# smarc-project/smarc_navigation

Measured on AMD Instinct MI355X. Metric: filter steps/sec at 1M particles x 512 MBES beams; pose RMSE vs ref, higher is better.
Workload: dtype f64 state / f32 ray-cast; 1 GPU; 1048576 particles/GPU x 512 beams, 999698-triangle mesh (708x708 height field triangulated) -- RECOGNISED AS A LATTICE by mesh_build: swept on its 708 x 708 node heights, no triangle record is read (an irregular TIN of the same size: value_tin / extra.mesh_tin), predict+MBES update+normalise+systematic resample+mean/cov per step; particles_per_gpu=1048576, beams=512, map=mesh, parallelism=particle-shard x1

## Files before the change

smarc_navigation_amd/csrc/mcl_api.hip:

```cpp
#include "mcl_host.h"
#include "mcl_host_resample.h"
#include "mcl_host_moments.h"
#include "mcl_host_update.h"
#include "mcl_host_landmarks.h"
#include "mcl_host_ranges.h"
#include "mcl_host_step.h"
#include "mcl_host_history.h"
#include "mcl_host_acoustic.h"
#include "mcl_recovery.h"


#include "mcl_dr_impl.h"
#include "mcl_gridmap.h"

extern "C" {

int mcl_abi_version(void) { return MCL_ABI_VERSION; }

const char* mcl_status_string(int s) {
  switch (s) {
    case MCL_OK: return "ok";
    case MCL_ERR_INVALID: return "invalid argument";
    case MCL_ERR_NO_DEVICE: return "no gfx950 HIP device";
    case MCL_ERR_HIP: return "HIP runtime error";
// ... 49 lines not shown
  h->world = cfg->world > 1 ? cfg->world : 1;
  h->rank = h->world > 1 ? cfg->rank : 0;
  h->ng = cfg->n_global > 0 ? cfg->n_global : cfg->n_particles;
  h->goff = h->world > 1 ? cfg->global_offset : 0;
  h->device = cfg->device;
  memset(&h->tacc, 0, sizeof h->tacc);
  {
    auto on = [](const char* name) {
      const char* v = getenv(name);
      return v && v[0] == '1';
    };
    auto env_tristate = [](const char* name) {
      const char* v = getenv(name);
      return !v ? -1 : (v[0] == '1' ? 1 : 0);
    };
    h->env_debug_work = getenv("MCL_DEBUG_WORK") != nullptr;
    h->env_sort = env_tristate("MCL_SORT_VISITS");
    h->env_sweep = env_tristate("MCL_SWEEP");
    h->env_slice = env_tristate("MCL_SLICE");
    h->env_slice_group = env_tristate("MCL_SLICE_GROUP");
    h->env_handover_slice = env_tristate("MCL_HANDOVER_SLICE");
    h->env_visit = env_tristate("MCL_VISIT");
    h->env_sweep_uniform = env_tristate("MCL_SWEEP_UNIFORM");
    if (const char* sv = getenv("MCL_SWEEP_STEP_CAP")) h->env_sweep_step_cap = std::max(0, atoi(sv));
    if (const char* sv = getenv("MCL_VISIT_BINS")) {
      int b[3] = {0, 0, 0};
      if (sscanf(sv, "%d,%d,%d", &b[0], &b[1], &b[2]) == 3 && b[0] >= 1 && b[1] >= 1 && b[2] >= 1 &&
          (long long)b[0] * b[1] * b[2] <= VISIT_MAX_BINS && (b[0] * b[1] * b[2]) % 64 == 0)
        for (int c = 0; c < 3; ++c) h->visit_nb[c] = b[c];
    }
    if (const char* sv = getenv("MCL_VISIT_RANGE")) {
      const double r = atof(sv);
      if (r >= 0.5 && r <= 16.0) h->visit_range = (float)r;
    }
    if (const char* sv = getenv("MCL_VISIT_MIN_N")) h->visit_min_n = std::max(1ll, atoll(sv));
    if (const char* sv = getenv("MCL_SWEEP_NSUB")) h->env_nsub = (sv[0] == '2' || sv[0] == '4') ? sv[0] - '0' : 1;
    h->env_force_comm = on("MCL_FORCE_COMM");
    if (const char* ex = getenv("MCL_EXCHANGE")) h->exch_allgather = strcmp(ex, "allgather") == 0;
    if (const char* fi = getenv("MCL_FAULT_INJECT")) h->fault_step = strcmp(fi, "step_after_predict") == 0;
    h->env_no_overlap = on("MCL_NO_OVERLAP");
  }
  if (h->ng > 0xffffffffll || h->goff + h->n > h->ng || h->rank >= h->world) {
    g_create_err = "mcl_create: inconsistent shard geometry";
    delete h;
    return MCL_ERR_INVALID;
  }
// ... 1185 lines not shown
```

smarc_navigation_amd/csrc/mcl_host.h:

```cpp
#pragma once
#include <hip/hip_runtime.h>
#include <rccl/rccl.h>

#include <rocprim/device/device_radix_sort.hpp>

#include <chrono>
#include <cmath>
#include <cstdlib>
#include <cstdio>
#include <cstring>
#include <string>
#include <thread>
#include <vector>

#include "../../include/mcl.h"
#include "mcl_host_pure.h"
#include "mcl_kernels.h"
#include "mcl_mbes.h"
#include "mcl_sweep.h"
#include "mcl_slice.h"
#include "mcl_mesh.h"
#include "mcl_resample.h"
#include "mcl_resample_alt.h"
#include "mcl_landmarks.h"
// ... 84 lines not shown
  DevBuf<int> dupes;
  DevBuf<double> cs, chunk, uni_dev;
  long long residual_k = -1;
  bool idx_explicit = false;
  int beams_cap = 0;
  std::vector<float> beam_cache;
  int beam_lo = -1, beam_hi = -1;
  bool beams_sorted = false;
  std::vector<float> ranges_host;
  bool sweep_angles_ok = false;
  int b_split = 0;
  int sweep_cap = 0;
  DevBuf<float> sweep_buf[2];
  PinBuf<float> sweep_stage[2];
  hipEvent_t ev_stage[2] = {nullptr, nullptr};
  bool stage_used[2] = {false, false};
  int sweep_sel = 0;
  hipStream_t copy_stream = nullptr;
  DevBuf<u32> defer_idx;
  DevBuf<u32> defer2_idx;
  int env_handover_slice = -1;
  int env_sweep_step_cap = 0;
  int env_sweep_uniform = -1;
  DevBuf<unsigned long long> sweep_work_dev;
  DevBuf<unsigned> reasons_dev;
  DevBuf<u32> visit_okey, visit_base;
  DevBuf<unsigned short> visit_cnt;
  DevBuf<u64> visit_desc;
  u32 visit_epoch = 0;
  DevBuf<VisitPar> visit_par;
  unsigned visit_flip = 0;
  bool gather_attr_set = false;
  bool visit_ready = false;
  bool pose_visit = false;
  int env_visit = -1;
  int visit_nb[3] = {16, 32, 8};
  float visit_range = 2.5f;
  long long visit_min_n = 393216;
  int env_sweep = -1;
  int env_nsub = 0;
  bool sweep_now = false;
  bool slice_now = false;
  bool handover_slice_now = false;
  int env_slice = -1;
  int env_slice_group = -1;
  DevBuf<u32> slice_loose;
// ... 287 lines not shown
```

smarc_navigation_amd/csrc/mcl_host_update.h:

```cpp
#pragma once
#include "mcl_host_moments.h"

namespace {

int upload_beams(mcl_handle* h, const float* ranges, const float* beam_angles, int B) {
  h->det_ride = nullptr;
  h->det_ride_dev = nullptr;
  if (B > h->beams_cap) {
    h->beams_cap = 0;
    h->beam_cache.clear();
    RESERVE(h, h->beam_sc, (size_t)B);
    RESERVE(h, h->ranges_dev, (size_t)B);
    h->beams_cap = B;
  }
  if ((int)h->beam_cache.size() != B || memcmp(h->beam_cache.data(), beam_angles, sizeof(float) * B) != 0) {
    std::vector<float2> sc(B);
    for (int b = 0; b < B; ++b) {
      sc[b].x = (float)std::sin((double)beam_angles[b]);
      sc[b].y = (float)std::cos((double)beam_angles[b]);
    }
    RET_IF(upload(h, h->beam_sc, sc.data(), sizeof(float2) * (size_t)B));
    h->beam_cache.assign(beam_angles, beam_angles + B);
    int lo = 0, hi = 0;
    bool finite = true;
// ... 385 lines not shown
void cast_slice_handovers(mcl_handle* h, int dgrid, const MbesArgs& d) {
  k_mbes_cast<1, EXPECT, 2><<<dgrid, MBES_THREADS, 0, h->stream>>>(d);
}

int allow_slice_group_lds(mcl_handle* h, size_t lds_g) {
  if (h->slice_attr_set && lds_g <= h->slice_attr_bytes) return MCL_OK;
  HIPCHK(h, hipFuncSetAttribute((const void*)k_mbes_slice_group, hipFuncAttributeMaxDynamicSharedMemorySize, (int)lds_g));
  h->slice_attr_set = true;
  h->slice_attr_bytes = lds_g;
  return MCL_OK;
}

struct SweepGrid {
  int sgrid, sthreads, dgrid;
  size_t lds;
};

template <int SURF, int MAP>
void launch_sweep(mcl_handle* h, const MbesPlan& p, const SweepGrid& g, const MbesArgs& a, const MbesArgs& d) {
  if (p.with_ranges) {
    t_begin(h, MCL_K_MBES_MAIN);
    if (p.nsub > 1)
      k_mbes_sweep<SURF, false, true><<<g.sgrid, g.sthreads, g.lds, h->stream>>>(a);
    else if ((SURF == 2 || SURF == 3) && a.sweep_work)
      k_mbes_sweep_work<(SURF == 3 ? 3 : 2)><<<g.sgrid, SWEEP_THREADS, g.lds, h->stream>>>(a);
    else
      k_mbes_sweep<SURF, false><<<g.sgrid, SWEEP_THREADS, g.lds, h->stream>>>(a);
    t_end(h);
    k_mbes_cast<MAP, false, 2><<<g.dgrid, MBES_THREADS, 0, h->stream>>>(d);
  } else {
    k_mbes_sweep<SURF, true><<<g.sgrid, SWEEP_THREADS, g.lds, h->stream>>>(a);
    k_mbes_cast<MAP, true, 2><<<g.dgrid, MBES_THREADS, 0, h->stream>>>(d);
  }
}

bool staged_handover(const mcl_handle* h, const MbesPlan& p) {
  return p.with_ranges && p.nsub == 1 && h->map_kind == 1 && !p.structured && h->mesh->tin_holes && h->mesh->cell_tri &&
         h->env_slice != 0 && h->env_handover_slice != 0;
}
int run_staged_handover(mcl_handle* h, const MbesPlan& p, const SweepGrid& g, const MbesArgs& a, MbesArgs d, const MbesCounters& wh) {
  const int B = p.B;
  RESERVE(h, h->defer2_idx, (size_t)h->n);
  const long long ngr = (h->n + SLICE_G - 1) / SLICE_G;
  RESERVE(h, h->slice_loose, (size_t)ngr);
  t_begin(h, MCL_K_MBES_MAIN);
  if (h->mesh->tin_rims)
    k_mbes_sweep<6, false><<<g.sgrid, SWEEP_THREADS, g.lds, h->stream>>>(a);
  else
// ... 18 lines not shown
    s2.slice_loose_count = (int*)(h->ctrl + CTRL_LOOSE);
    k_mbes_slice_group<<<(unsigned)std::min<long long>(ngr, hgrid), SLICE_G_THREADS, lds_g, h->stream>>>(s2);
  }
  k_mbes_slice<false><<<pgrid, SLICE_THREADS, slice_lds_bytes(B), h->stream>>>(s2);
  d.perm = h->defer2_idx;
  d.n_dev = s2.defer_count;
  cast_slice_handovers<false>(h, g.dgrid, d);
  return MCL_OK;
}

void debug_sweep_handovers(mcl_handle* h, const MbesArgs& a) {
  int cnt = 0;
  (void)hipMemcpyAsync(&cnt, a.defer_count, sizeof(int), hipMemcpyDeviceToHost, h->stream);
  (void)hipStreamSynchronize(h->stream);
  unsigned long long shared = 0, steps = 0;
  if (a.sweep_work) {
    unsigned long long w[64];
    (void)hipMemcpy(w, a.sweep_work, sizeof w, hipMemcpyDeviceToHost);
    for (int k = 0; k < 64; ++k) {
      shared += w[k] >> 32;
      steps += w[k] & 0xffffffffull;
    }
  }
  fprintf(stderr, "[mbes] sweep handed over %d of %lld particles (clamp to r_max %s); wave walk steps shared %llu of %llu\n", cnt,
          (long long)h->n, a.sweep_noclamp ? "proved idle: skipped" : "kept", shared, steps);
#ifdef SWEEP_REASONS
  unsigned why[16];
  (void)hipMemcpy(why, h->reasons_dev, sizeof why, hipMemcpyDeviceToHost);
  (void)hipMemset(h->reasons_dev, 0, sizeof why);
  fprintf(stderr, "[mbes] declined sides by reason:");
  for (int k = 0; k < 16; ++k)
    if (why[k]) fprintf(stderr, " %d:%u", k, why[k]);
  fprintf(stderr, "\n");
#endif
}

int run_sweep(mcl_handle* h, const MbesPlan& p, MbesArgs& a, const MbesCounters& wh) {
  a.sweep_noclamp = sweep_noclamp(h, p) ? 1 : 0;
  a.sweep_uniform = h->env_sweep_uniform == 1 ? 1 : 0;
  a.sweep_step_cap = h->env_sweep_step_cap;
  a.sweep_work = nullptr;
  if (h->env_debug_work) {
    RESERVE(h, h->sweep_work_dev, 64);
    HIPCHK(h, hipMemsetAsync(h->sweep_work_dev, 0, 64 * sizeof(unsigned long long), h->stream));
    a.sweep_work = h->sweep_work_dev;
  }
  SweepGrid g;
  g.sthreads = p.nsub == 4 ? 512 : SWEEP_THREADS;
  const int per_block = g.sthreads / 64 / (2 * p.nsub) * 64;
  g.sgrid = (int)((p.n_part + per_block - 1) / per_block);
  g.lds = sweep_lds_bytes(p.B);
  g.dgrid = handover_cast_grid(p, wh);
  const MbesArgs d = handover_cast_args(a, wh);
  const bool staged = staged_handover(h, p);
  if (p.with_ranges) h->handover_slice_now = staged;
  if (staged)
    RET_IF(run_staged_handover(h, p, g, a, d, wh));
  else if (h->map_kind == 0)
    launch_sweep<0, 0>(h, p, g, a, d);
  else if (!p.structured && h->mesh->tin_rims)
    launch_sweep<6, 1>(h, p, g, a, d);
  else if (!p.structured)
    launch_sweep<5, 1>(h, p, g, a, d);
// ... 223 lines not shown
```

smarc_navigation_amd/csrc/mcl_mbes.h:

```cpp
#pragma once
#include <hip/hip_fp16.h>

#include "mcl_device.h"
#include "mcl_kernels.h"

#ifndef MBES_WAVES
#define MBES_WAVES 8
#endif
#ifndef MBES_MIN_WAVES_PER_SIMD
#define MBES_MIN_WAVES_PER_SIMD 8
#endif
#ifndef MBES_MIN_WAVES_MESH
#define MBES_MIN_WAVES_MESH 6
#endif
#define MBES_THREADS (MBES_WAVES * 64)
#ifndef MBES_TILE_FLOATS
#define MBES_TILE_FLOATS 8192
#endif
#ifndef MBES_DIR_BINS
#define MBES_DIR_BINS 16
#endif
#ifndef MBES_DIR_BINS
#define MBES_DIR_BINS 16
#endif
// ... 26 lines not shown
  u32 tin_he_bytes;
  const u32* cell_rim;
  u32 tin_outline;
  u32 tin_nhe;
  const float4* cell_tri;
  double x0, y0;
};

struct MbesArgs {
  const double* st[6];
  long long n;
  double m2o[12];
  double off_t[3];
  double off_R[9];
  MbesPose* pose;
  const float2* beam_sc;
  const float* ranges;
  int n_beams;
  int sorted;
  int b_lo, b_hi;
  const float* grid;
  const float* grid_pad;
  int nyp;
  int nx, ny;
  double ox, oy, inv_res;
  float res;
  float zmin_map, zmax_map;
  int cells;
  int diag_mode;
  float inv_sigma, r_max;
  double lognorm;
  double* lw;
  u64* max_slots;
  float* exp_out;
  long long exp_first, exp_count;
  MeshArgs mesh;
  const u32* perm;
  struct MbesGroup* groups;
  int* worklist;
  int* work_count;
  unsigned long long* stats;
  const float4* sweep_beams;
  const float* sweep_tail_run;
  const float* sweep_tan0;
  const float* sweep_tail;
  int b_split;
// ... 891 lines not shown
```

smarc_navigation_amd/csrc/mcl_mesh.h:

```cpp
#pragma once
#include <algorithm>
#include <cmath>
#include <cstring>
#include <string>
#include <unordered_map>
#include <vector>

#include "../../include/mcl.h"
#include "mcl_halfedge.h"
#include "mcl_mbes.h"

struct MeshDev {
  DevBuf<float4> tri;
  DevBuf<float4> tri_mt;
  DevBuf<u32> cell_start;
  DevBuf<uint2> cell_info;
  int gx = 0, gy = 0;
  double x0 = 0, y0 = 0, cs = 1;
  float zmin = 0, zmax = 0;
  size_t n_records = 0;
  DevBuf<float> heights;
  DevBuf<float> heights_pad;
  size_t n_vertical = 0;
  int diag_mode = 0;
  double slope_max = 0;
  DevBuf<uint4> tin_he;
  size_t tin_he_bytes = 0;
  bool tin_ok = false;
  size_t tin_nhe = 0;
  size_t tin_outline = 0;
  size_t tin_rims = 0;
  DevBuf<u32> cell_rim;
  bool tin_holes = false;
  DevBuf<float4> cell_tri;
};

inline size_t padded_heights_count(int nx, int ny) { return ((size_t)nx + 2) * ((size_t)ny + 2); }
inline hipError_t upload_padded_heights(const float* z, int nx, int ny, float* out) {
  const size_t nyp = (size_t)ny + 2, cnt = padded_heights_count(nx, ny);
  std::vector<float> pad(cnt);
  auto nanp = [](uint32_t payload) {
    const uint32_t b = 0x7fc00000u | payload;
    float f;
    memcpy(&f, &b, 4);
    return f;
  };
  for (size_t i = 0; i < (size_t)nx + 2; ++i)
    for (size_t j = 0; j < nyp; ++j) {
      const bool ox = i == 0 || i == (size_t)nx + 1, oy = j == 0 || j == nyp - 1;
      pad[i * nyp + j] = (ox || oy) ? nanp((ox ? 1u : 0u) | (oy ? 2u : 0u)) : z[(i - 1) * (size_t)ny + (j - 1)];
    }
  return hipMemcpy(out, pad.data(), sizeof(float) * cnt, hipMemcpyHostToDevice);
}

inline void mesh_free(MeshDev* m) { delete m; }

inline float half_bits_to_float(uint16_t h) {
  const uint32_t sign = (uint32_t)(h & 0x8000u) << 16, exp = (h >> 10) & 0x1fu, man = h & 0x3ffu;
  uint32_t bits;
  if (exp == 0) {
    if (man == 0) {
      bits = sign;
    } else {
      float f = (float)man * 5.9604644775390625e-08f;
      memcpy(&bits, &f, 4);
      bits |= sign;
    }
  } else if (exp == 31) {
    bits = sign | 0x7f800000u | (man << 13);
  } else {
    bits = sign | ((exp + 112u) << 23) | (man << 13);
  }
  float out;
  memcpy(&out, &bits, 4);
  return out;
// ... 373 lines not shown
            const u32 dbit = (ix < (size_t)m->gx && iy < (size_t)m->gy) ? diag[ix * m->gy + iy] : 0u;
            b = (b & ~1u) | dbit;
            memcpy(&hts[ix * nny + iy], &b, 4);
          }
      {
        double g2 = 0.0;
        for (size_t ix = 0; ix + 1 < nnx; ++ix)
          for (size_t iy = 0; iy + 1 < nny; ++iy) {
            const double h00 = hts[ix * nny + iy], h10 = hts[(ix + 1) * nny + iy], h01 = hts[ix * nny + iy + 1],
                         h11 = hts[(ix + 1) * nny + iy + 1];
            const double ax = std::max(std::fabs(h10 - h00), std::fabs(h11 - h01));
            const double ay = std::max(std::fabs(h01 - h00), std::fabs(h11 - h10));
            g2 = std::max(g2, ax * ax + ay * ay);
          }
        m->slope_max = std::sqrt(g2) / cs;
      }
      if (m->heights.reserve(hts.size()) != MCL_OK || m->heights_pad.reserve(padded_heights_count((int)nnx, (int)nny)) != MCL_OK ||
          hipMemcpy(m->heights, hts.data(), sizeof(float) * hts.size(), hipMemcpyHostToDevice) != hipSuccess ||
          upload_padded_heights(hts.data(), (int)nnx, (int)nny, m->heights_pad) != hipSuccess) {
        *err = "set_map_mesh: device allocation failed";
        mesh_free(m);
        return MCL_ERR_ALLOC;
      }
    }
  }
  if (!m->heights || want_slice) {
    std::vector<float4> ct(3 * std::max<size_t>(m->n_records, 1));
    for (size_t r = 0; r < m->n_records; ++r) {
      const u32 k = rec_tri[r];
      for (int c = 0; c < 3; ++c) {
        const float* v = verts + 3 * (size_t)tris[3 * (size_t)k + c];
        ct[3 * r + c] = make_float4(v[0], v[1], v[2], 0.f);
      }
      memcpy(&ct[3 * r].w, &k, 4);
    }
    if (m->cell_tri.reserve(ct.size()) != MCL_OK ||
        hipMemcpy(m->cell_tri, ct.data(), sizeof(float4) * ct.size(), hipMemcpyHostToDevice) != hipSuccess) {
      (void)hipGetLastError();
      m->cell_tri.reset();
    }
  }
  *out = m;
  return MCL_OK;
}

inline MeshArgs mesh_args(const MeshDev* m) {
// ... 19 lines not shown
```

smarc_navigation_amd/csrc/mcl_sweep.h:

```cpp
#pragma once
#include "mcl_halfedge.h"
#include "mcl_mbes.h"

#ifndef SWEEP_THREADS
#define SWEEP_THREADS 256
#endif
#ifndef SWEEP_MIN_WAVES_GRID
#define SWEEP_MIN_WAVES_GRID 6
#endif
#ifndef SWEEP_MIN_WAVES_TIN
#define SWEEP_MIN_WAVES_TIN 6
#endif
#define SWEEP_TIN_GAPS 12
#ifndef SWEEP_MIN_WAVES
#define SWEEP_MIN_WAVES 8
#endif

#ifdef SWEEP_REASONS
#define SWEEP_NOTE(code) do { if (a.reasons) atomicAdd(&a.reasons[(code) & 15], 1u); } while (0)
#else
#define SWEEP_NOTE(code) ((void)0)
#endif
#define SWEEP_FAIL(code) do { SWEEP_NOTE(code); return false; } while (0)
#ifdef SWEEP_TIMELINE
// ... 97 lines not shown
               : [acc] "+v"(acc), [bp] "+v"(bp),
                 [ep] "=&v"(ep), [d] "=&v"(d), [ec] "=&v"(ec), [e2] "=&v"(e2), [sav] "=&s"(sav), [odd] "=&s"(odd)
               : [dss] "v"(dss), [num] "v"(num), [tp] "v"(tp), [sc] "v"(sc), [tc] "v"(tc), [dts] "v"(dts), [sel] "s"(sel)
               : "vcc", "scc", "v56", "v57", "v58", "v59", "v60", "v61", "v62", "v63");
}

__device__ __forceinline__ float seg_tau(float num, float D, float tp, float tc) {
  return __builtin_amdgcn_fmed3f(num * __builtin_amdgcn_rcpf(D), tp, tc);
}

struct SweepNode {
  int P;
  float d;
  float s, t;
};

__device__ __forceinline__ bool sweep_border_final(const MbesArgs& a, float h, float c2z, float c1x, float c1y) {
  const unsigned side = __float_as_uint(h) & 3u;
  const float sb = fast_sqrt(fmaxf(1.f - c2z * c2z, 0.f));
  const float lhs = sb * (a.sweep_slope + sb), rhs = 0.9f * (c2z - a.sweep_slope * sb);
  return (side == 1u || side == 2u) & (lhs < rhs * fabsf(side == 1u ? c1x : c1y));
}

template <int SURF, bool EXPECT_ONLY, bool SUB = false, bool WORK = false>
__device__ __forceinline__ bool sweep_side(const MbesArgs& a, const MbesPose& P, const float4* __restrict__ sbeam,
                                           const float* __restrict__ stail, int side, int sub, int nsub,
                                           float* __restrict__ exp_row, float& acc_out) {
  acc_out = 0.f;
  const int nx = a.nx, ny = a.ny, B = a.n_beams;
  bool pre = P.um >= 1.0 && P.um < (double)(nx - 2) && P.vm >= 1.0 && P.vm < (double)(ny - 2);
  const float c2z = P.c2[2];
  pre = pre & (c2z >= a.sweep_c2z_min);
  const double fum = pre ? floor(P.um) : 1.0, fvm = pre ? floor(P.vm) : 1.0;
  const int I0 = (int)fum, J0 = (int)fvm;
  const float ul = (float)(P.um - fum), vl = (float)(P.vm - fvm);
  const float res = a.res, inv_res = (float)a.inv_res, oz = P.oz;
  const float sg = side ? -1.f : 1.f;
  const int nb_side = side ? a.b_split : B - a.b_split;
  const int per = SUB ? max((nb_side + nsub - 1) / nsub, 2) : nb_side;
  const int first = SUB ? min(sub * per, nb_side) : 0, last = SUB ? min(first + per, nb_side) : nb_side;
  int ptr = side ? a.b_split - 1 - first : a.b_split + first;
  const int pstep = side ? -1 : 1, pend = side ? a.b_split - 1 - last : a.b_split + last;
  const bool none = ptr == pend;
  float s_stop = none ? 0.f : a.r_max;
  if (!none) {
    const float2 sc = a.beam_sc[side ? 0 : B - 1];
    const float dz_e = sc.x * P.c1[2] - sc.y * c2z;
    if (dz_e < -1e-4f) s_stop = fminf(s_stop, (a.zmin_map - oz) * fast_rcp(dz_e) * fabsf(sc.x));
  }
  s_stop += 2.f * res;
  {
    const float rc = fast_rcp(c2z);
    const float sl = fabsf(P.c1[2]) * (s_stop + 2.f * res);
    const float t_hi = ((oz - a.zmin_map) + sl) * rc + res, t_lo = fminf(((oz - a.zmax_map) - sl) * rc - res, 0.f);
    const float s_hi = s_stop + 2.f * res;
    const float ax = sg * P.c1[0] * inv_res, ay = sg * P.c1[1] * inv_res, bx = -P.c2[0] * inv_res, by = -P.c2[1] * inv_res;
    const float fi0 = (float)I0, fj0 = (float)J0;
    const float n0 = fminf(t_lo * bx, t_hi * bx), n1 = fmaxf(t_lo * bx, t_hi * bx);
    const float m0 = fminf(t_lo * by, t_hi * by), m1 = fmaxf(t_lo * by, t_hi * by);
    pre = pre & (fi0 + n0 >= 3.f) & (fi0 + n1 <= (float)(nx - 5)) & (fj0 + m0 >= 3.f) & (fj0 + m1 <= (float)(ny - 5));
    pre = pre & (s_hi * fmaxf(fabsf(ax), fabsf(ay)) + fmaxf(-t_lo, t_hi) * fmaxf(fabsf(bx), fabsf(by)) < 30000.f);
  }
  if (!pre) SWEEP_FAIL(1);
  const int nyp = a.nyp;
  const int g0i = (I0 + 1) * nyp + (J0 + 1);
  const float* __restrict__ gp = a.grid_pad + (size_t)g0i;
  const __amdgpu_buffer_rsrc_t grsrc = __builtin_amdgcn_make_buffer_rsrc((void*)a.grid_pad, 0, (nx + 2) * nyp * 4, 0x00020000);
  const int ny4 = nyp * 4, g0b = g0i * 4;
  float dxs = -P.c2[0], dys = -P.c2[1], dzs = -c2z, r0 = 0.f;
  bool own_start = false;
  if (SUB && first > 0 && !none) {
    const float2 sc = a.beam_sc[ptr];
    dxs = sc.x * P.c1[0] - sc.y * P.c2[0];
    dys = sc.x * P.c1[1] - sc.y * P.c2[1];
    dzs = sc.x * P.c1[2] - sc.y * c2z;
    const float te = dzs < -1e-4f ? fminf(a.r_max, (a.zmin_map - oz) * fast_rcp(dzs) + res) : a.r_max;
    const float ex = te * dxs * inv_res, ey = te * dys * inv_res;
    own_start = ((float)I0 + fminf(ex, 0.f) >= 3.f) & ((float)I0 + fmaxf(ex, 0.f) <= (float)(nx - 5)) &
                ((float)J0 + fminf(ey, 0.f) >= 3.f) & ((float)J0 + fmaxf(ey, 0.f) <= (float)(ny - 5));
    if (!own_start) {
      dxs = -P.c2[0];
      dys = -P.c2[1];
      dzs = -c2z;
    }
  }
  for (int attempt = 0; attempt < 2; ++attempt) {
    r0 = cast_clear<SURF>(gp, nyp, a, ul, vl, oz, dxs * inv_res, dys * inv_res, dzs, a.zmax_map, a.r_max);
    if (!SUB || !own_start || ((r0 < a.r_max) & (r0 > 0.f))) break;
    dxs = -P.c2[0];
    dys = -P.c2[1];
    dzs = -c2z;
    own_start = false;
  }
  if (!(r0 < a.r_max)) SWEEP_FAIL(5);
  if (none) return true;
  const float nx_ = P.c1[1] * P.c2[2] - P.c1[2] * P.c2[1], ny_ = P.c1[2] * P.c2[0] - P.c1[0] * P.c2[2],
              nz_ = P.c1[0] * P.c2[1] - P.c1[1] * P.c2[0];
  const float pu = nx_ * res, pv = ny_ * res, pz = nz_, p0 = -(pu * ul + pv * vl + pz * oz);
  const float su = sg * P.c1[0] * res, sv = sg * P.c1[1] * res, sz = sg * P.c1[2];
  float s0 = -(su * ul + sv * vl + sz * oz);
  const float tu = -P.c2[0] * res, tv = -P.c2[1] * res, tz = -c2z, t0 = -(tu * ul + tv * vl + tz * oz);
  auto node = [&](int Pk) {
    SweepNode N;
    N.P = Pk;
    const int j = __builtin_amdgcn_sbfe(Pk, 0, 16), i = (Pk - j) >> 16;
    const float h = gp[i * nyp + j];
    const float fi = (float)i, fj = (float)j;
    N.d = fmaf(pu, fi, fmaf(pv, fj, fmaf(pz, h, p0)));
    N.s = fmaf(su, fi, fmaf(sv, fj, fmaf(sz, h, s0)));
    N.t = fmaf(tu, fi, fmaf(tv, fj, fmaf(tz, h, t0)));
    return N;
  };
  SweepNode A, Bn;
  int C;
  float s_prev, t_prev, s_cur, t_cur;
  {
    const float uh = fmaf(r0, dxs * inv_res, ul), vh = fmaf(r0, dys * inv_res, vl);
    const float cfi = floorf(uh), cfj = floorf(vh);
    const float fu = uh - cfi, fv = vh - cfj;
    const int c00 = (int)cfi * 65536 + (int)cfj;
    int k0, k1, k2;
    if (SURF == 2) {
      const bool lower = fv <= fu;
      k0 = c00;
      k1 = lower ? c00 + 65536 : c00 + 65537;
      k2 = lower ? c00 + 65537 : c00 + 1;
    } else {
      const bool lower = fu + fv <= 1.f;
      k0 = lower ? c00 : c00 + 65536;
      k1 = lower ? c00 + 65536 : c00 + 65537;
// ... 48 lines not shown
      sweep_merge_asm(msel, acc, bp, dss, num, tp, sc, tc, dts);
    } else {
      while (e_cur >= 0.f && (!SUB || bp != bp_end)) {
        const float tau = seg_tau(num, fmaf(-tcur, dts, dss), tp, tc);
        if (EXPECT_ONLY) {
          exp_row[(int)(bp - sb_off) >> 4] = fminf(tau * bm.y, a.r_max);
        } else {
          const float dd = hw_max(fmaf(-tau, bm.y, bm.z), bm.w);
          acc = fmaf(dd, dd, acc);
        }
        tcur = bm.x;
        bp += pstep16;
        const float4 r = sbeam[(int)(bp - sb_off) >> 4];
        bm.x = r.x;
        bm.y = r.y;
        bm.z = r.z;
        bm.w = r.w;
        e_cur = fmaf(-tcur, tc, sc);
      }
    }
  };
  const auto walk_step = [&](float& sp, float& tp, float& sc, float& tc, const int step, auto EXITS) -> bool {
    const int Nk = (int)((unsigned)A.P + (unsigned)Bn.P - (unsigned)C);
    const int nj = __builtin_amdgcn_sbfe(Nk, 0, 16), ni = (Nk - nj) >> 16;
    const float hN = __int_as_float(__builtin_amdgcn_raw_buffer_load_b32(grsrc, __mul24(ni, ny4) + ((nj << 2) + g0b), 0, 0));
    const float dts = tc - tp;
    const float dss = sc - sp, num = fmaf(tp, dss, -(sp * dts));
    merge_segment(sp, tp, sc, tc, dts, dss, num);
    if (decltype(EXITS)::value) {
      if (bp == bp_end) return true;
      if (sc > s_stop) return true;
      if (step > max_steps) {
        SWEEP_NOTE(11);
        ok = false;
        return true;
      }
    }
    const float fi = (float)ni, fj = (float)nj;
    const float dN = fmaf(pu, fi, fmaf(pv, fj, fmaf(pz, hN, p0)));
    const bool keep_a = (__float_as_int(dN) ^ __float_as_int(A.d)) < 0;
    C = keep_a ? Bn.P : A.P;
    Bn.P = keep_a ? A.P : Bn.P;
    Bn.d = keep_a ? A.d : Bn.d;
    Bn.s = keep_a ? A.s : Bn.s;
    Bn.t = keep_a ? A.t : Bn.t;
    A.P = Nk;
    A.d = dN;
    A.s = fmaf(su, fi, fmaf(sv, fj, fmaf(sz, hN, s0)));
    A.t = fmaf(tu, fi, fmaf(tv, fj, fmaf(tz, hN, t0)));
    const float lam = A.d * fast_rcp(A.d - Bn.d);
    const float s_new = fmaf(lam, Bn.s - A.s, A.s), t_new = fmaf(lam, Bn.t - A.t, A.t);
    sp = s_new;
    tp = t_new;
    if (!(t_new > 0.f)) {
      ok = false;
      return true;
    }
    return false;
  };
  const auto lane_walk = [&](int step, bool mid) -> int {
    for (;; step += 2) {
      if (!mid && walk_step(s_prev, t_prev, s_cur, t_cur, step, std::true_type())) break;
      mid = false;
      if (walk_step(s_cur, t_cur, s_prev, t_prev, step + 1, std::false_type())) return WORK ? step + 1 : 0;
    }
    return WORK ? step : 0;
  };
  if (!EXPECT_ONLY && !SUB) {
    int uA = __builtin_amdgcn_readfirstlane(A.P), uB = __builtin_amdgcn_readfirstlane(Bn.P), uC = __builtin_amdgcn_readfirstlane(C);
    const int ug0b = __builtin_amdgcn_readfirstlane(g0b);
    const bool same = (A.P == uA) & (Bn.P == uB) & (C == uC) & (g0b == ug0b);
    const bool gate = a.sweep_uniform && __builtin_amdgcn_ballot_w64(same) == __builtin_amdgcn_ballot_w64(true);
    unsigned long long fin_m = 0ull, ok_m = ~0ull;
    const auto shared_step = [&](float& sp, float& tp, float& sc, float& tc, const int step, auto EXITS) -> bool {
      const int Nk = (int)((unsigned)uA + (unsigned)uB - (unsigned)uC);
      const int nj = (int)(short)Nk, ni = (Nk - nj) >> 16;
      const float hN = __int_as_float(__builtin_amdgcn_raw_buffer_load_b32(grsrc, ni * ny4 + ((nj << 2) + ug0b), 0, 0));
      const float dts = tc - tp;
      const float dss = sc - sp, num = fmaf(tp, dss, -(sp * dts));
      merge_segment(sp, tp, sc, tc, dts, dss, num);
      unsigned long long out_m = fin_m, over_m = 0ull;
      if (decltype(EXITS)::value) {
        out_m |= __builtin_amdgcn_ballot_w64(bp == bp_end) | __builtin_amdgcn_ballot_w64(sc > s_stop);
        over_m = __builtin_amdgcn_ballot_w64(step > max_steps) & ~out_m;
#ifdef SWEEP_REASONS
        if (__builtin_amdgcn_inverse_ballot_w64(over_m)) SWEEP_NOTE(11);
#endif
        out_m |= over_m;
      }
      const int uA_was = uA;
      const float fi = (float)ni, fj = (float)nj;
// ... 44 lines not shown
        if (shared_step(s_cur, t_cur, s_prev, t_prev, step + 1, std::false_type())) break;
        how = 3;
        if ((__builtin_amdgcn_ballot_w64(true) & ~fin_m) == 0ull) break;
      }
    }
    const int n_shared = gate ? step + (how > 2 ? 1 : 0) : 0;
    const bool fin = __builtin_amdgcn_inverse_ballot_w64(fin_m);
    ok = __builtin_amdgcn_inverse_ballot_w64(ok_m);
    int n_steps = n_shared;
    if ((how & 1) == 0 && !fin) n_steps = lane_walk(how == 2 ? step : step + 2, how == 2);
    if (WORK && a.sweep_work) {
      const unsigned long long act = __builtin_amdgcn_ballot_w64(true);
      int wn = n_shared;
      for (unsigned long long m = act; m; m &= m - 1ull) wn = max(wn, __builtin_amdgcn_readlane(n_steps, (int)__builtin_ctzll(m)));
      const unsigned wave = blockIdx.x * (blockDim.x >> 6) + (threadIdx.x >> 6);
      if ((int)(threadIdx.x & 63) == (int)__builtin_ctzll(act))
        atomicAdd(&a.sweep_work[wave & 63u], ((unsigned long long)n_shared << 32) | (unsigned long long)wn);
    }
  } else {
    lane_walk(1, false);
  }
  if (!ok) {
    const int lj = __builtin_amdgcn_sbfe(A.P, 0, 16), li = (A.P - lj) >> 16;
    const float hN = __int_as_float(__builtin_amdgcn_raw_buffer_load_b32(grsrc, __mul24(li, ny4) + ((lj << 2) + g0b), 0, 0));
    ok = (hN != hN) && sweep_border_final(a, hN, c2z, su * inv_res, sv * inv_res);
    if (!ok) SWEEP_NOTE(hN != hN ? 10 : 12);
  }
  if (ok && bp != bp_end) {
    ptr = (int)(bp - sb_off) >> 4;
    if (EXPECT_ONLY) {
      for (; ptr != pend; ptr += pstep) exp_row[ptr] = a.r_max;
    } else {
      acc += stail[ptr];
    }
  }
  acc_out = acc;
  return ok;
}

template <bool EXPECT_ONLY, bool SUB = false>
__device__ __forceinline__ bool sweep_side_grid(const MbesArgs& a, const MbesPose& P, const float4* __restrict__ sbeam,
                                                const float* __restrict__ stail, int side, int sub, int nsub,
                                                float* __restrict__ exp_row, float& acc_out) {
  acc_out = 0.f;
  const int nx = a.nx, ny = a.ny, B = a.n_beams;
  bool pre = P.um >= 1.0 && P.um < (double)(nx - 2) && P.vm >= 1.0 && P.vm < (double)(ny - 2);
  const float c2z = P.c2[2];
// ... 637 lines not shown
    }
    return cross(hq, hb, sp, tp);
  };
  if (!(HOLES && blind)) {
    for (int step = 1;; step += 2) {
      if (walk_step(s_prev, t_prev, s_cur, t_cur, step, std::true_type())) break;
      if (walk_step(s_cur, t_cur, s_prev, t_prev, step + 1, std::false_type())) break;
    }
  }
  if (ok && bp != bp_end) {
    ptr = (int)(bp - sb_off) >> 4;
    if (EXPECT_ONLY) {
      for (; ptr != pend; ptr += pstep) exp_row[ptr] = a.r_max;
    } else {
      acc += stail[ptr];
    }
  }
  acc_out = acc;
  return ok;
}

#define SWEEP_MAX_WAVES 8

template <int SURF, bool EXPECT_ONLY, bool SUB, bool WORK>
__device__ __forceinline__ double sweep_lane(const MbesArgs& a, long long j0, long long n, const float4* sbeam,
                                             const float* stail, float* xacc, int* xok) {
  const int lane = threadIdx.x & 63, w = __builtin_amdgcn_readfirstlane((int)(threadIdx.x >> 6));
  const int nsub = SUB ? a.sweep_nsub : 1, combos = 2 * nsub;
  const int group = w / combos, combo = w - group * combos;
  const int side = combo & 1, sub = combo >> 1, pl = group * 64 + lane;
  const long long i = j0 + pl + (EXPECT_ONLY ? a.exp_first : 0);
  const bool valid = i < n;
  bool ok = true, work = valid;
  float* exp_row = nullptr;
  if (EXPECT_ONLY) {
    work = valid && i < a.exp_first + a.exp_count;
    if (work) exp_row = a.exp_out + (size_t)(i - a.exp_first) * a.n_beams;
  }
  float acc = 0.f;
  u32 slot = (u32)i;
  const float4* sside = sbeam + (side ? 0 : 2);
  if (work) {
    const MbesPose P = a.pose[i];
    slot = EXPECT_ONLY ? (u32)i : P.slot;
    if (SURF == 5 || SURF == 6)
      ok = sweep_side_tin<EXPECT_ONLY, SUB, SURF == 6>(a, P, sside, stail, side, sub, nsub, exp_row, acc);
    else if (SURF == 0)
      ok = sweep_side_grid<EXPECT_ONLY, SUB>(a, P, sside, stail, side, sub, nsub, exp_row, acc);
    else
      ok = sweep_side<(SURF == 3 ? 3 : 2), EXPECT_ONLY, SUB, WORK>(a, P, sside, stail, side, sub, nsub, exp_row, acc);
  }
  if (combo) {
    xacc[w * 64 + lane] = acc;
    xok[w * 64 + lane] = ok ? 1 : 0;
  }
#ifdef SWEEP_TIMELINE
  if (lane == 0 && blockIdx.x * (blockDim.x >> 6) + w < SWEEP_TL_WAVES)
    g_sweep_tl[6 * (blockIdx.x * (blockDim.x >> 6) + w) + 1] = wall_clock64();
#endif
  __syncthreads();
  double v = -__builtin_inf();
  if (!combo) {
    bool ok2 = ok;
    double acc2 = (double)acc;
    for (int c = 1; c < combos; ++c) {
      ok2 = ok2 & (xok[(w + c) * 64 + lane] != 0);
      acc2 += (double)xacc[(w + c) * 64 + lane];
    }
    if (work && ok2 && !EXPECT_ONLY) {
      v = -0.5 * acc2 - (double)a.sweep_nvalid * a.lognorm;
      a.lw[slot] = v;
    }
    const unsigned long long dm = __ballot(work && !ok2);
    if (dm) {
      int base = 0;
      if (lane == 0) base = atomicAdd(a.defer_count, (int)__popcll(dm));
      base = __builtin_amdgcn_readfirstlane(base);
      if (work && !ok2) a.defer_idx[base + (int)__popcll(dm & ((1ull << lane) - 1ull))] = (u32)i;
    }
  }
  return v == v ? v : -__builtin_inf();
}

inline size_t sweep_lds_bytes(int B) { return (size_t)(B + 7) * sizeof(float4) + (size_t)(B + 4) * sizeof(float); }

template <int SURF, bool EXPECT_ONLY, bool SUB, bool WORK>
__device__ __forceinline__ void sweep_kernel(const MbesArgs& a) {
#ifdef SWEEP_TIMELINE
  const unsigned long long tl0 = wall_clock64(), tc0 = __builtin_readcyclecounter();
#endif
  extern __shared__ __attribute__((aligned(16))) unsigned char sweep_lds[];
  __shared__ float xacc[64 * (SUB ? SWEEP_MAX_WAVES : SWEEP_THREADS / 64)];
  __shared__ int xok[64 * (SUB ? SWEEP_MAX_WAVES : SWEEP_THREADS / 64)];
  float4* sbeam = (float4*)sweep_lds + 4;
  float* stail = (float*)(sbeam + a.n_beams + 3);
  for (int b = threadIdx.x; b < a.n_beams; b += blockDim.x) {
    sbeam[b + (b >= a.b_split ? 2 : 0)] = a.sweep_beams[b];
    stail[b] = SUB ? a.sweep_tail_run[b] : a.sweep_tail[b];
  }
  if (threadIdx.x < 4) stail[a.n_beams + threadIdx.x] = a.sweep_tan0[threadIdx.x];
  if (threadIdx.x == 0) sbeam[-1] = sbeam[a.n_beams + 2] = make_float4(__builtin_inff(), 0.f, 0.f, 0.f);
  if (threadIdx.x == 1) sbeam[a.b_split] = make_float4(a.sweep_tan0[1], 0.f, 0.f, 0.f);
  if (threadIdx.x == 2) sbeam[a.b_split + 1] = make_float4(a.sweep_tan0[0], 0.f, 0.f, 0.f);
  __syncthreads();
  const int per_block = (int)(blockDim.x >> 6) / (2 * (SUB ? a.sweep_nsub : 1)) * 64;
  const double vmax = sweep_lane<SURF, EXPECT_ONLY, SUB, WORK>(a, blockIdx.x * (long long)per_block, a.n, sbeam, stail, xacc, xok);
  if (!EXPECT_ONLY && a.max_slots) {
    const double m = wave_max(vmax);
    if ((threadIdx.x & 63) == 0 && m > -__builtin_inf())
      atomicMax((unsigned long long*)&a.max_slots[(blockIdx.x * (blockDim.x >> 6) + (threadIdx.x >> 6)) & (MCL_MAX_SLOTS - 1)],
                ordered_key(m));
  }
#ifdef SWEEP_TIMELINE
  {
    const unsigned wv = blockIdx.x * (blockDim.x >> 6) + (threadIdx.x >> 6);
    if ((threadIdx.x & 63) == 0 && wv < SWEEP_TL_WAVES) {
      g_sweep_tl[6 * wv] = tl0;
      g_sweep_tl[6 * wv + 2] = wall_clock64();
      g_sweep_tl[6 * wv + 4] = tc0;
      g_sweep_tl[6 * wv + 5] = __builtin_readcyclecounter();
      g_sweep_tl[6 * wv + 3] = (unsigned long long)__builtin_amdgcn_s_getreg((31 << 11) | 4)
                               | ((unsigned long long)__builtin_amdgcn_s_getreg((31 << 11) | 20) << 32);
    }
  }
#endif
}

template <int SURF, bool EXPECT_ONLY, bool SUB = false>
__global__ void __launch_bounds__(SUB ? 64 * SWEEP_MAX_WAVES : SWEEP_THREADS, SURF == 0 ? (SUB ? SWEEP_MIN_WAVES_GRID - 1 : SWEEP_MIN_WAVES_GRID) : (SURF == 6 && !SUB && !EXPECT_ONLY ? 8 : (SURF == 5 || SURF == 6 ? SWEEP_MIN_WAVES_TIN : SWEEP_MIN_WAVES))) k_mbes_sweep(MbesArgs a) {
  sweep_kernel<SURF, EXPECT_ONLY, SUB, false>(a);
}
template <int SURF>
__global__ void __launch_bounds__(SWEEP_THREADS, SWEEP_MIN_WAVES) k_mbes_sweep_work(MbesArgs a) {
  sweep_kernel<SURF, false, false, true>(a);
}
```

Measured before the change: 2628 steps/s.

## Walk lattice sweep on padded float4 node records instead of height lookups

Builds a padded float4 table per lattice node holding height plus its i/j indices, and lets the structured sweep walk address nodes by byte offset. Each walk step then reads height and coordinates in one 96-bit buffer load, with no index unpacking or int-to-float conversion. The wave-uniform shared-walk path is bypassed when nodes are used. The node table is four times larger than the height array, which means more cache and memory traffic per step. It also adds another kernel variant and a host-side table build.

```diff
diff --git a/smarc_navigation_amd/csrc/mcl_api.hip b/smarc_navigation_amd/csrc/mcl_api.hip
--- a/smarc_navigation_amd/csrc/mcl_api.hip
+++ b/smarc_navigation_amd/csrc/mcl_api.hip
@@ -95,6 +95,7 @@
     h->env_handover_slice = env_tristate("MCL_HANDOVER_SLICE");
     h->env_visit = env_tristate("MCL_VISIT");
     h->env_sweep_uniform = env_tristate("MCL_SWEEP_UNIFORM");
+    h->env_sweep_nodes = env_tristate("MCL_SWEEP_NODES");
     if (const char* sv = getenv("MCL_SWEEP_STEP_CAP")) h->env_sweep_step_cap = std::max(0, atoi(sv));
     if (const char* sv = getenv("MCL_VISIT_BINS")) {
       int b[3] = {0, 0, 0};
diff --git a/smarc_navigation_amd/csrc/mcl_host.h b/smarc_navigation_amd/csrc/mcl_host.h
--- a/smarc_navigation_amd/csrc/mcl_host.h
+++ b/smarc_navigation_amd/csrc/mcl_host.h
@@ -130,6 +130,7 @@
   int env_handover_slice = -1;
   int env_sweep_step_cap = 0;
   int env_sweep_uniform = -1;
+  int env_sweep_nodes = -1;
   DevBuf<unsigned long long> sweep_work_dev;
   DevBuf<unsigned> reasons_dev;
   DevBuf<u32> visit_okey, visit_base;
diff --git a/smarc_navigation_amd/csrc/mcl_host_update.h b/smarc_navigation_amd/csrc/mcl_host_update.h
--- a/smarc_navigation_amd/csrc/mcl_host_update.h
+++ b/smarc_navigation_amd/csrc/mcl_host_update.h
@@ -431,8 +431,12 @@
     t_begin(h, MCL_K_MBES_MAIN);
     if (p.nsub > 1)
       k_mbes_sweep<SURF, false, true><<<g.sgrid, g.sthreads, g.lds, h->stream>>>(a);
+    else if ((SURF == 2 || SURF == 3) && a.sweep_work && a.node_tab)
+      k_mbes_sweep_work<(SURF == 3 ? 3 : 2), true><<<g.sgrid, SWEEP_THREADS, g.lds, h->stream>>>(a);
     else if ((SURF == 2 || SURF == 3) && a.sweep_work)
-      k_mbes_sweep_work<(SURF == 3 ? 3 : 2)><<<g.sgrid, SWEEP_THREADS, g.lds, h->stream>>>(a);
+      k_mbes_sweep_work<(SURF == 3 ? 3 : 2), false><<<g.sgrid, SWEEP_THREADS, g.lds, h->stream>>>(a);
+    else if ((SURF == 2 || SURF == 3) && !a.node_tab)
+      k_mbes_sweep_heights<(SURF == 3 ? 3 : 2)><<<g.sgrid, SWEEP_THREADS, g.lds, h->stream>>>(a);
     else
       k_mbes_sweep<SURF, false><<<g.sgrid, SWEEP_THREADS, g.lds, h->stream>>>(a);
     t_end(h);
@@ -497,8 +501,8 @@
       steps += w[k] & 0xffffffffull;
     }
   }
-  fprintf(stderr, "[mbes] sweep handed over %d of %lld particles (clamp to r_max %s); wave walk steps shared %llu of %llu\n", cnt,
-          (long long)h->n, a.sweep_noclamp ? "proved idle: skipped" : "kept", shared, steps);
+  fprintf(stderr, "[mbes] sweep handed over %d of %lld particles (clamp to r_max %s); wave walk steps shared %llu of %llu; lattice walk on %s\n", cnt,
+          (long long)h->n, a.sweep_noclamp ? "proved idle: skipped" : "kept", shared, steps, a.node_tab ? "node records" : "heights");
 #ifdef SWEEP_REASONS
   unsigned why[16];
   (void)hipMemcpy(why, h->reasons_dev, sizeof why, hipMemcpyDeviceToHost);
@@ -510,10 +514,22 @@
 #endif
 }
 
+bool sweep_nodes(const mcl_handle* h, const MbesPlan& p) {
+  return h->map_kind == 1 && p.structured && (p.args.diag_mode == 1 || p.args.diag_mode == 2) && p.with_ranges && p.nsub == 1 &&
+         h->env_sweep_nodes != 0 && h->env_sweep_uniform != 1 && h->mesh->nodes_pad &&
+         node_table_fits(p.args.nx, p.args.ny);
+}
+
 int run_sweep(mcl_handle* h, const MbesPlan& p, MbesArgs& a, const MbesCounters& wh) {
   a.sweep_noclamp = sweep_noclamp(h, p) ? 1 : 0;
   a.sweep_uniform = h->env_sweep_uniform == 1 ? 1 : 0;
   a.sweep_step_cap = h->env_sweep_step_cap;
+  a.node_tab = nullptr;
+  a.node_bytes = 0;
+  if (sweep_nodes(h, p)) {
+    a.node_tab = h->mesh->nodes_pad;
+    a.node_bytes = (unsigned)(padded_heights_count(a.nx, a.ny) * sizeof(float4));
+  }
   a.sweep_work = nullptr;
   if (h->env_debug_work) {
     RESERVE(h, h->sweep_work_dev, 64);
diff --git a/smarc_navigation_amd/csrc/mcl_mbes.h b/smarc_navigation_amd/csrc/mcl_mbes.h
--- a/smarc_navigation_amd/csrc/mcl_mbes.h
+++ b/smarc_navigation_amd/csrc/mcl_mbes.h
@@ -72,6 +72,8 @@
   const float* grid;
   const float* grid_pad;
   int nyp;
+  const float4* node_tab;
+  unsigned node_bytes;
   int nx, ny;
   double ox, oy, inv_res;
   float res;
diff --git a/smarc_navigation_amd/csrc/mcl_mesh.h b/smarc_navigation_amd/csrc/mcl_mesh.h
--- a/smarc_navigation_amd/csrc/mcl_mesh.h
+++ b/smarc_navigation_amd/csrc/mcl_mesh.h
@@ -21,6 +21,7 @@
   size_t n_records = 0;
   DevBuf<float> heights;
   DevBuf<float> heights_pad;
+  DevBuf<float4> nodes_pad;
   size_t n_vertical = 0;
   int diag_mode = 0;
   double slope_max = 0;
@@ -51,6 +52,25 @@
       pad[i * nyp + j] = (ox || oy) ? nanp((ox ? 1u : 0u) | (oy ? 2u : 0u)) : z[(i - 1) * (size_t)ny + (j - 1)];
     }
   return hipMemcpy(out, pad.data(), sizeof(float) * cnt, hipMemcpyHostToDevice);
+}
+
+inline bool node_table_fits(int nx, int ny) { return padded_heights_count(nx, ny) * sizeof(float4) < ((size_t)1 << 31); }
+inline hipError_t upload_node_table(const float* z, int nx, int ny, float4* out) {
+  const size_t nyp = (size_t)ny + 2, cnt = padded_heights_count(nx, ny);
+  std::vector<float4> tab(cnt);
+  auto nanp = [](uint32_t payload) {
+    const uint32_t b = 0x7fc00000u | payload;
+    float f;
+    memcpy(&f, &b, 4);
+    return f;
+  };
+  for (size_t i = 0; i < (size_t)nx + 2; ++i)
+    for (size_t j = 0; j < nyp; ++j) {
+      const bool ox = i == 0 || i == (size_t)nx + 1, oy = j == 0 || j == nyp - 1;
+      const float h = (ox || oy) ? nanp((ox ? 1u : 0u) | (oy ? 2u : 0u)) : z[(i - 1) * (size_t)ny + (j - 1)];
+      tab[i * nyp + j] = make_float4(h, (float)((long long)i - 1), (float)((long long)j - 1), 0.f);
+    }
+  return hipMemcpy(out, tab.data(), sizeof(float4) * cnt, hipMemcpyHostToDevice);
 }
 
 inline void mesh_free(MeshDev* m) { delete m; }
@@ -470,6 +490,13 @@
         mesh_free(m);
         return MCL_ERR_ALLOC;
       }
+      if (m->diag_mode != 0 && node_table_fits((int)nnx, (int)nny)) {
+        if (m->nodes_pad.reserve(padded_heights_count((int)nnx, (int)nny)) != MCL_OK ||
+            upload_node_table(hts.data(), (int)nnx, (int)nny, m->nodes_pad) != hipSuccess) {
+          (void)hipGetLastError();
+          m->nodes_pad.reset();
+        }
+      }
     }
   }
   if (!m->heights || want_slice) {
diff --git a/smarc_navigation_amd/csrc/mcl_sweep.h b/smarc_navigation_amd/csrc/mcl_sweep.h
--- a/smarc_navigation_amd/csrc/mcl_sweep.h
+++ b/smarc_navigation_amd/csrc/mcl_sweep.h
@@ -143,7 +143,7 @@
   return (side == 1u || side == 2u) & (lhs < rhs * fabsf(side == 1u ? c1x : c1y));
 }
 
-template <int SURF, bool EXPECT_ONLY, bool SUB = false, bool WORK = false>
+template <int SURF, bool EXPECT_ONLY, bool SUB = false, bool WORK = false, bool NODES = false>
 __device__ __forceinline__ bool sweep_side(const MbesArgs& a, const MbesPose& P, const float4* __restrict__ sbeam,
                                            const float* __restrict__ stail, int side, int sub, int nsub,
                                            float* __restrict__ exp_row, float& acc_out) {
@@ -188,6 +188,10 @@
   const float* __restrict__ gp = a.grid_pad + (size_t)g0i;
   const __amdgpu_buffer_rsrc_t grsrc = __builtin_amdgcn_make_buffer_rsrc((void*)a.grid_pad, 0, (nx + 2) * nyp * 4, 0x00020000);
   const int ny4 = nyp * 4, g0b = g0i * 4;
+  const __amdgpu_buffer_rsrc_t nrsrc = __builtin_amdgcn_make_buffer_rsrc((void*)(NODES ? (const void*)a.node_tab : (const void*)a.grid_pad), 0, NODES ? (int)a.node_bytes : 0, 0x00020000);
+  const int ny16 = nyp * 16, g0n = g0i * 16;
+  const float fI0 = (float)I0, fJ0 = (float)J0;
+  typedef int sweep_i3 __attribute__((ext_vector_type(3)));
   float dxs = -P.c2[0], dys = -P.c2[1], dzs = -c2z, r0 = 0.f;
   bool own_start = false;
   if (SUB && first > 0 && !none) {
@@ -223,10 +227,20 @@
   const float tu = -P.c2[0] * res, tv = -P.c2[1] * res, tz = -c2z, t0 = -(tu * ul + tv * vl + tz * oz);
   auto node = [&](int Pk) {
     SweepNode N;
-    N.P = Pk;
     const int j = __builtin_amdgcn_sbfe(Pk, 0, 16), i = (Pk - j) >> 16;
-    const float h = gp[i * nyp + j];
-    const float fi = (float)i, fj = (float)j;
+    float h, fi, fj;
+    if (NODES) {
+      N.P = g0n + i * ny16 + j * 16;
+      const sweep_i3 rec = __builtin_amdgcn_raw_buffer_load_b96(nrsrc, N.P, 0, 0);
+      h = __int_as_float(rec.x);
+      fi = __int_as_float(rec.y) - fI0;
+      fj = __int_as_float(rec.z) - fJ0;
+    } else {
+      N.P = Pk;
+      h = gp[i * nyp + j];
+      fi = (float)i;
+      fj = (float)j;
+    }
     N.d = fmaf(pu, fi, fmaf(pv, fj, fmaf(pz, h, p0)));
     N.s = fmaf(su, fi, fmaf(sv, fj, fmaf(sz, h, s0)));
     N.t = fmaf(tu, fi, fmaf(tv, fj, fmaf(tz, h, t0)));
@@ -321,8 +335,17 @@
   };
   const auto walk_step = [&](float& sp, float& tp, float& sc, float& tc, const int step, auto EXITS) -> bool {
     const int Nk = (int)((unsigned)A.P + (unsigned)Bn.P - (unsigned)C);
-    const int nj = __builtin_amdgcn_sbfe(Nk, 0, 16), ni = (Nk - nj) >> 16;
-    const float hN = __int_as_float(__builtin_amdgcn_raw_buffer_load_b32(grsrc, __mul24(ni, ny4) + ((nj << 2) + g0b), 0, 0));
+    int nj = 0, ni = 0;
+    float hN, fni = 0.f, fnj = 0.f;
+    if (NODES) {
+      const sweep_i3 rec = __builtin_amdgcn_raw_buffer_load_b96(nrsrc, Nk, 0, 0);
+      hN = __int_as_float(rec.x);
+      fni = __int_as_float(rec.y);
+      fnj = __int_as_float(rec.z);
+    } else {
+      nj = __builtin_amdgcn_sbfe(Nk, 0, 16), ni = (Nk - nj) >> 16;
+      hN = __int_as_float(__builtin_amdgcn_raw_buffer_load_b32(grsrc, __mul24(ni, ny4) + ((nj << 2) + g0b), 0, 0));
+    }
     const float dts = tc - tp;
     const float dss = sc - sp, num = fmaf(tp, dss, -(sp * dts));
     merge_segment(sp, tp, sc, tc, dts, dss, num);
@@ -335,7 +358,7 @@
         return true;
       }
     }
-    const float fi = (float)ni, fj = (float)nj;
+    const float fi = NODES ? fni - fI0 : (float)ni, fj = NODES ? fnj - fJ0 : (float)nj;
     const float dN = fmaf(pu, fi, fmaf(pv, fj, fmaf(pz, hN, p0)));
     const bool keep_a = (__float_as_int(dN) ^ __float_as_int(A.d)) < 0;
     C = keep_a ? Bn.P : A.P;
@@ -365,7 +388,16 @@
     }
     return WORK ? step : 0;
   };
-  if (!EXPECT_ONLY && !SUB) {
+  if (NODES) {
+    const int n_steps = lane_walk(1, false);
+    if (WORK && a.sweep_work) {
+      const unsigned long long act = __builtin_amdgcn_ballot_w64(true);
+      int wn = 0;
+      for (unsigned long long m = act; m; m &= m - 1ull) wn = max(wn, __builtin_amdgcn_readlane(n_steps, (int)__builtin_ctzll(m)));
+      const unsigned wave = blockIdx.x * (blockDim.x >> 6) + (threadIdx.x >> 6);
+      if ((int)(threadIdx.x & 63) == (int)__builtin_ctzll(act)) atomicAdd(&a.sweep_work[wave & 63u], (unsigned long long)wn);
+    }
+  } else if (!EXPECT_ONLY && !SUB) {
     int uA = __builtin_amdgcn_readfirstlane(A.P), uB = __builtin_amdgcn_readfirstlane(Bn.P), uC = __builtin_amdgcn_readfirstlane(C);
     const int ug0b = __builtin_amdgcn_readfirstlane(g0b);
     const bool same = (A.P == uA) & (Bn.P == uB) & (C == uC) & (g0b == ug0b);
@@ -456,7 +488,8 @@
   }
   if (!ok) {
     const int lj = __builtin_amdgcn_sbfe(A.P, 0, 16), li = (A.P - lj) >> 16;
-    const float hN = __int_as_float(__builtin_amdgcn_raw_buffer_load_b32(grsrc, __mul24(li, ny4) + ((lj << 2) + g0b), 0, 0));
+    const float hN = __int_as_float(NODES ? __builtin_amdgcn_raw_buffer_load_b32(nrsrc, A.P, 0, 0)
+                                          : __builtin_amdgcn_raw_buffer_load_b32(grsrc, __mul24(li, ny4) + ((lj << 2) + g0b), 0, 0));
     ok = (hN != hN) && sweep_border_final(a, hN, c2z, su * inv_res, sv * inv_res);
     if (!ok) SWEEP_NOTE(hN != hN ? 10 : 12);
   }
@@ -1140,7 +1173,7 @@
 
 #define SWEEP_MAX_WAVES 8
 
-template <int SURF, bool EXPECT_ONLY, bool SUB, bool WORK>
+template <int SURF, bool EXPECT_ONLY, bool SUB, bool WORK, bool NODES>
 __device__ __forceinline__ double sweep_lane(const MbesArgs& a, long long j0, long long n, const float4* sbeam,
                                              const float* stail, float* xacc, int* xok) {
   const int lane = threadIdx.x & 63, w = __builtin_amdgcn_readfirstlane((int)(threadIdx.x >> 6));
@@ -1166,7 +1199,7 @@
     else if (SURF == 0)
       ok = sweep_side_grid<EXPECT_ONLY, SUB>(a, P, sside, stail, side, sub, nsub, exp_row, acc);
     else
-      ok = sweep_side<(SURF == 3 ? 3 : 2), EXPECT_ONLY, SUB, WORK>(a, P, sside, stail, side, sub, nsub, exp_row, acc);
+      ok = sweep_side<(SURF == 3 ? 3 : 2), EXPECT_ONLY, SUB, WORK, NODES>(a, P, sside, stail, side, sub, nsub, exp_row, acc);
   }
   if (combo) {
     xacc[w * 64 + lane] = acc;
@@ -1202,7 +1235,7 @@
 
 inline size_t sweep_lds_bytes(int B) { return (size_t)(B + 7) * sizeof(float4) + (size_t)(B + 4) * sizeof(float); }
 
-template <int SURF, bool EXPECT_ONLY, bool SUB, bool WORK>
+template <int SURF, bool EXPECT_ONLY, bool SUB, bool WORK, bool NODES>
 __device__ __forceinline__ void sweep_kernel(const MbesArgs& a) {
 #ifdef SWEEP_TIMELINE
   const unsigned long long tl0 = wall_clock64(), tc0 = __builtin_readcyclecounter();
@@ -1222,7 +1255,7 @@
   if (threadIdx.x == 2) sbeam[a.b_split + 1] = make_float4(a.sweep_tan0[0], 0.f, 0.f, 0.f);
   __syncthreads();
   const int per_block = (int)(blockDim.x >> 6) / (2 * (SUB ? a.sweep_nsub : 1)) * 64;
-  const double vmax = sweep_lane<SURF, EXPECT_ONLY, SUB, WORK>(a, blockIdx.x * (long long)per_block, a.n, sbeam, stail, xacc, xok);
+  const double vmax = sweep_lane<SURF, EXPECT_ONLY, SUB, WORK, NODES>(a, blockIdx.x * (long long)per_block, a.n, sbeam, stail, xacc, xok);
   if (!EXPECT_ONLY && a.max_slots) {
     const double m = wave_max(vmax);
     if ((threadIdx.x & 63) == 0 && m > -__builtin_inf())
@@ -1246,9 +1279,13 @@
 
 template <int SURF, bool EXPECT_ONLY, bool SUB = false>
 __global__ void __launch_bounds__(SUB ? 64 * SWEEP_MAX_WAVES : SWEEP_THREADS, SURF == 0 ? (SUB ? SWEEP_MIN_WAVES_GRID - 1 : SWEEP_MIN_WAVES_GRID) : (SURF == 6 && !SUB && !EXPECT_ONLY ? 8 : (SURF == 5 || SURF == 6 ? SWEEP_MIN_WAVES_TIN : SWEEP_MIN_WAVES))) k_mbes_sweep(MbesArgs a) {
-  sweep_kernel<SURF, EXPECT_ONLY, SUB, false>(a);
+  sweep_kernel<SURF, EXPECT_ONLY, SUB, false, (SURF == 2 || SURF == 3) && !EXPECT_ONLY && !SUB>(a);
 }
 template <int SURF>
+__global__ void __launch_bounds__(SWEEP_THREADS, SWEEP_MIN_WAVES) k_mbes_sweep_heights(MbesArgs a) {
+  sweep_kernel<SURF, false, false, false, false>(a);
+}
+template <int SURF, bool NODES>
 __global__ void __launch_bounds__(SWEEP_THREADS, SWEEP_MIN_WAVES) k_mbes_sweep_work(MbesArgs a) {
-  sweep_kernel<SURF, false, false, true>(a);
+  sweep_kernel<SURF, false, false, true, NODES>(a);
 }
```

After: 2601 steps/s. 0.99x the previous value.
